# ZeayW/Multimodal-fusion-based-Pre-routing-Timing-Prediction-

Hardware: AMD Instinct MI355X
Metric: train-step samples/sec (higher is better)
Workload: dtype bf16; 1 GPU; config B: 8 designs/step/GPU, 65536-node netlist, 64 levels, 256x256 tile, 1350 endpoints/design, UNet(max), bf16 operands / fp32 accumulate on the MFMA-bound contractions; U-Net activations and their gradients stored bf16, netlist tensors, statistics, parameters and gradients fp32; nodes=65536, levels=64, tile=256, endpoints_per_design=1350, cone_pruning=False, parallelism=dp1 (designs sharded, one all-reduce of the flat gradient per step), launch=one HIP graph replay per step (Adam inside)

## Files before the change

multimodal-fusion-based-pre-routing-timing-prediction-_amd/csrc/mlp2_bf16.hip:

```cpp
#include <stdlib.h>
#include "mlp_tile_bf16.h"
#include "fold_gather.h"

namespace mmft {

constexpr int L2_BM = 32;

struct Mlp2Bf16Args {
  const float* x1;
  long long ldx1;
  const int* rows;
  int n;
  const unsigned short* w1;
  const float* b1;
  const unsigned short* w2;
  const float* b2;
  const float* mask;
  long long ldmask;
  float* hid_out;
  long long ldhid;
  int hid16;
  float* out;
  long long ldout;
  int add_act, relu_out;
  const unsigned char* active;
};

__global__ void __launch_bounds__(512) mlp2_rows_bf16_kernel(Mlp2Bf16Args a) {
  __shared__ __attribute__((aligned(16))) unsigned short xs[L2_BM * L2_XS];
  __shared__ __attribute__((aligned(16))) unsigned short hs[L2_BM * L2_HS];
  const int tid = threadIdx.x, lane = tid & 63, wave = tid >> 6;
  const int m0 = blockIdx.x * L2_BM;
  auto live_row = [&](int r) -> bool { return m0 + r < a.n && (!a.active || a.active[a.rows[m0 + r]]); };
  if (a.active) {
    int any = 0;
    if (tid < L2_BM) any = live_row(tid) ? 1 : 0;
    if (!__syncthreads_or(any)) return;
  }
  const int r16 = lane & 15, q = lane >> 4;

  bf16x8 w1f[2][4], w2f[8];
  load_w1_frags(w1f, a.w1, wave, r16, q);
  load_w2_frags(w2f, a.w2, wave, r16, q);
  {
    const int r = tid >> 4, k8 = (tid & 15) * 8;
    f32x4 v0 = {0.f, 0.f, 0.f, 0.f}, v1 = v0;
    if (live_row(r)) {
      const float* p = a.x1 + (long long)a.rows[m0 + r] * a.ldx1 + k8;
      v0 = *reinterpret_cast<const f32x4*>(p);
      v1 = *reinterpret_cast<const f32x4*>(p + 4);
    }
    u32x4 pk = {pack_bf16(v0.x, v0.y), pack_bf16(v0.z, v0.w), pack_bf16(v1.x, v1.y), pack_bf16(v1.z, v1.w)};
    *reinterpret_cast<u32x4*>(xs + r * L2_XS + k8) = pk;
  }
  __syncthreads();

  f32x4 acc1[2][2];
  tile_layer1<4, 2>(acc1, w1f, xs, L2_XS, r16, q);
#pragma unroll
  for (int i = 0; i < 2; ++i)
#pragma unroll
    for (int j = 0; j < 2; ++j) {
      const int m = i * 16 + r16, nn = wave * 32 + j * 16 + q * 4;
      f32x4 v = acc1[i][j];
      const bool live = live_row(m);
      const long long row = live ? (long long)a.rows[m0 + m] : 0;
      if (a.mask) {
        f32x4 mk = {0.f, 0.f, 0.f, 0.f};
        if (live) mk = hid_load4(a.mask, row * a.ldmask + nn, a.hid16);
        v = relu_mask4(v, mk);
      } else {
        if (a.b1) v += *reinterpret_cast<const f32x4*>(a.b1 + nn);
        v = relu4(v);
      }
      st_bf16x4(hs + m * L2_HS + nn, v);
      if (a.hid_out && live) hid_store4(a.hid_out, row * a.ldhid + nn, v, a.hid16);
    }
  __syncthreads();

  f32x4 acc2[2];
#pragma unroll
  for (int i = 0; i < 2; ++i) acc2[i] = tile_layer2(w2f, hs, L2_HS, r16, q, i);
#pragma unroll
  for (int i = 0; i < 2; ++i) {
    const int m = i * 16 + r16;
    if (!live_row(m)) continue;
    const int nn = wave * 16 + q * 4;
    float* o = a.out + (long long)a.rows[m0 + m] * a.ldout + nn;
    f32x4 v = acc2[i];
    if (a.b2) v += *reinterpret_cast<const f32x4*>(a.b2 + nn);
    if (a.add_act) v += *reinterpret_cast<const f32x4*>(o);
    if (a.relu_out) v = relu4(v);
    *reinterpret_cast<f32x4*>(o) = v;
  }
}

template <bool KEEP>
struct Kept {};
template <>
struct Kept<true> {
  float *A, *LSE;
  float* hid_out;
  long long ldhid;
  int hid16;
};

struct LevelFwdCommon {
  float* h;
  const float* pre;
  long long ld;
  const int *in_ptr, *in_idx, *ic_ptr, *ic_idx, *ic_drv;
  int net_row0, n_net;
  const int* rows;
  int cell_row0, n_cell;
  const unsigned short *w1, *w2;
  const float *b1, *b2;
  int relu;
  const unsigned char* active;
  int cell_tiles;
};

template <bool KEEP>
struct LevelFwdArgs : LevelFwdCommon, Kept<KEEP> {};

template <bool KEEP>
__global__ void __launch_bounds__(512) level_fwd_bf16_kernel(LevelFwdArgs<KEEP> a) {
  constexpr int BM = 16;
  __shared__ __attribute__((aligned(16))) unsigned short xs[BM * L2_XS];
  __shared__ __attribute__((aligned(16))) unsigned short hs[BM * L2_HS];
  const int tid = threadIdx.x, lane = tid & 63, wave = tid >> 6;
  const FoldSrc fs{a.h, a.pre, a.ld, a.in_ptr, a.in_idx, a.ic_idx, a.ic_drv, a.net_row0, a.n_net, a.relu};
  if ((int)blockIdx.x >= a.cell_tiles) {
    const long long total = (long long)a.n_net * 32;
    for (long long t = (long long)(blockIdx.x - a.cell_tiles) * 512 + tid; t < total;
         t += (long long)(gridDim.x - a.cell_tiles) * 512) {
      const int u = a.net_row0 + (int)(t >> 5), c = ((int)t & 31) * 4;
      if (a.active && !a.active[u]) continue;
      *reinterpret_cast<f32x4*>(a.h + (long long)u * a.ld + c) = fold_net_value(fs, u, c);
    }
    return;
  }
  const int m0 = blockIdx.x * BM;
  auto row_of = [&](int r) -> int { return a.rows ? a.rows[m0 + r] : a.cell_row0 + m0 + r; };
  auto live_row = [&](int r) -> bool { return m0 + r < a.n_cell && (!a.active || a.active[row_of(r)]); };
  if (a.active) {
    int any = 0;
    if (tid < BM) any = live_row(tid) ? 1 : 0;
    if (!__syncthreads_or(any)) return;
  }
  const int r16 = lane & 15, q = lane >> 4;
  bf16x8 w1f[2][4], w2f[8];
  load_w1_frags(w1f, a.w1, wave, r16, q);

  {
    const int r = tid >> 5, c = (tid & 31) * 4;
    f32x4 av = {0.f, 0.f, 0.f, 0.f};
    if (live_row(r)) {
      const int v = row_of(r);
      const int e0 = a.ic_ptr[v], e1 = a.ic_ptr[v + 1];
      SoftAccT<true> sa;
      sa.init();
      fold_gather_edges(fs, e0, e1, 1, c, sa);
      [[maybe_unused]] f32x4 lv = {0.f, 0.f, 0.f, 0.f};
      if (e1 > e0) {
#pragma unroll
        for (int j = 0; j < 4; ++j) {
          av[j] = sa.acc[j] / sa.s[j];
          if constexpr (KEEP) lv[j] = sa.mx[j] + fg_log<true>(sa.s[j]);
        }
      }
      if constexpr (KEEP) {
        *reinterpret_cast<f32x4*>(a.A + (long long)v * a.ld + c) = av;
        *reinterpret_cast<f32x4*>(a.LSE + (long long)v * a.ld + c) = lv;
      }
    }
    st_bf16x4(xs + r * L2_XS + c, av);
  }
  load_w2_frags(w2f, a.w2, wave, r16, q);
  __syncthreads();

  f32x4 acc1[1][2];
  tile_layer1<4, 1>(acc1, w1f, xs, L2_XS, r16, q);
#pragma unroll
  for (int j = 0; j < 2; ++j) {
    const int nn = wave * 32 + j * 16 + q * 4;
    f32x4 v = acc1[0][j];
    if (a.b1) v += *reinterpret_cast<const f32x4*>(a.b1 + nn);
    v = relu4(v);
    st_bf16x4(hs + r16 * L2_HS + nn, v);
    if constexpr (KEEP) {
      if (a.hid_out && live_row(r16)) hid_store4(a.hid_out, (long long)row_of(r16) * a.ldhid + nn, v, a.hid16);
    }
  }
  __syncthreads();
  if (!live_row(r16)) return;
  const int nn = wave * 16 + q * 4;
  float* o = a.h + (long long)row_of(r16) * a.ld + nn;
  f32x4 v = tile_layer2(w2f, hs, L2_HS, r16, q, 0);
  if (a.b2) v += *reinterpret_cast<const f32x4*>(a.b2 + nn);
  v += *reinterpret_cast<const f32x4*>(o);
  if (a.relu) v = relu4(v);
  *reinterpret_cast<f32x4*>(o) = v;
}

struct LevelSlotsCommon {
  float* h;
  const float* pre;
  long long ld;
  const int* slots;
  const int* net_drv;
  int net_row0, n_net, cell_row0, n_cell;
  const unsigned short *w1, *w2;
  const float *b1, *b2;
  int relu;
  const unsigned char* active;
  int cell_tiles;
};

template <bool KEEP>
struct LevelSlotsArgs : LevelSlotsCommon, Kept<KEEP> {};

template <int RB, bool KEEP>
__global__ void __launch_bounds__(512) level_fwd_slots_kernel(LevelSlotsArgs<KEEP> a) {
  constexpr int BM = 16 * RB;
  __shared__ __attribute__((aligned(16))) unsigned short xs[BM * L2_XS];
  __shared__ __attribute__((aligned(16))) unsigned short hs[BM * L2_HS];
  const int tid = threadIdx.x, lane = tid & 63, wave = tid >> 6;
  const int r16 = lane & 15, q = lane >> 4;
  const int b = blockIdx.x, gr = tid >> 5, gc = (tid & 31) * 4;
  const bool has_cell = b < a.cell_tiles;
  const int m0 = b * BM;
  int nd[RB];
  f32x4 npre[RB];
  bool net_ok[RB], live[RB];
  int hrow[RB][4], prow[RB][4];
#pragma unroll
  for (int rb = 0; rb < RB; ++rb) {
    const int nrow = b * BM + gr + 16 * rb, u = a.net_row0 + nrow;
    net_ok[rb] = nrow < a.n_net && (!a.active || a.active[u]);
    nd[rb] = -1;
    npre[rb] = f32x4{0.f, 0.f, 0.f, 0.f};
    if (net_ok[rb]) {
      nd[rb] = a.net_drv[u];
      npre[rb] = *reinterpret_cast<const f32x4*>(a.pre + (long long)u * a.ld + gc);
    }
    const int v = a.cell_row0 + m0 + gr + 16 * rb;
    live[rb] = has_cell && m0 + gr + 16 * rb < a.n_cell && (!a.active || a.active[v]);
#pragma unroll
    for (int k = 0; k < 4; ++k) hrow[rb][k] = prow[rb][k] = -1;
    if (live[rb]) {
      const int4 s0 = *reinterpret_cast<const int4*>(a.slots + (long long)v * 8);
      const int4 s1 = *reinterpret_cast<const int4*>(a.slots + (long long)v * 8 + 4);
      hrow[rb][0] = s0.x; hrow[rb][1] = s0.y; hrow[rb][2] = s0.z; hrow[rb][3] = s0.w;
      prow[rb][0] = s1.x; prow[rb][1] = s1.y; prow[rb][2] = s1.z; prow[rb][3] = s1.w;
    }
  }
  bf16x8 w1f[2][4], w2f[8];
  bool elive[RB];
  f32x4 hold[RB];
#pragma unroll
  for (int rb = 0; rb < RB; ++rb) {
    const int ev = a.cell_row0 + m0 + r16 + 16 * rb;
    elive[rb] = has_cell && m0 + r16 + 16 * rb < a.n_cell && (!a.active || a.active[ev]);
    hold[rb] = f32x4{0.f, 0.f, 0.f, 0.f};
  }
  if (has_cell) {
    load_w1_frags(w1f, a.w1, wave, r16, q);
#pragma unroll
    for (int rb = 0; rb < RB; ++rb)
      if (elive[rb]) hold[rb] = *reinterpret_cast<const f32x4*>(a.h + (long long)(a.cell_row0 + m0 + r16 + 16 * rb) * a.ld + wave * 16 + q * 4);
  }
#pragma unroll
  for (int rb = 0; rb < RB; ++rb)
    if (net_ok[rb]) {
      const int u = a.net_row0 + b * BM + gr + 16 * rb;
      f32x4 hd = {0.f, 0.f, 0.f, 0.f};
      if (nd[rb] >= 0) hd = *reinterpret_cast<const f32x4*>(a.h + (long long)nd[rb] * a.ld + gc);
      *reinterpret_cast<f32x4*>(a.h + (long long)u * a.ld + gc) = fg_finish_net(hd, npre[rb], a.relu);
    }
  if (!has_cell) return;
  if (a.active) {
    int any = 0;
    if (tid < BM) any = (m0 + tid < a.n_cell && a.active[a.cell_row0 + m0 + tid]) ? 1 : 0;
    if (!__syncthreads_or(any)) return;
  }
#pragma unroll
  for (int rb = 0; rb < RB; ++rb) {
    const int v = a.cell_row0 + m0 + gr + 16 * rb;
    f32x4 av = {0.f, 0.f, 0.f, 0.f};
    if (live[rb]) {
      const int h0 = hrow[rb][0] >= 0 ? hrow[rb][0] : v;
      f32x4 xa[4], xp[4];
#pragma unroll
      for (int k = 0; k < 4; ++k) {
        xa[k] = *reinterpret_cast<const f32x4*>(a.h + (long long)(hrow[rb][k] >= 0 ? hrow[rb][k] : h0) * a.ld + gc);
        xp[k] = *reinterpret_cast<const f32x4*>(a.pre + (long long)(prow[rb][k] >= 0 ? prow[rb][k] : a.net_row0) * a.ld + gc);
      }
      SoftAccT<true> sa;
      sa.init();
#pragma unroll
      for (int k = 0; k < 4; ++k) {
        const f32x4 x = prow[rb][k] >= 0 ? fg_finish_net(xa[k], xp[k], a.relu) : xa[k];
        SoftAccT<true> nx = sa;
        nx.add(x);
        const bool ok = hrow[rb][k] >= 0;
#pragma unroll
        for (int j = 0; j < 4; ++j) {
          sa.mx[j] = ok ? nx.mx[j] : sa.mx[j];
          sa.s[j] = ok ? nx.s[j] : sa.s[j];
          sa.acc[j] = ok ? nx.acc[j] : sa.acc[j];
        }
      }
      [[maybe_unused]] f32x4 lv = {0.f, 0.f, 0.f, 0.f};
      if (hrow[rb][0] >= 0) {
#pragma unroll
        for (int j = 0; j < 4; ++j) {
          av[j] = sa.acc[j] / sa.s[j];
          if constexpr (KEEP) lv[j] = sa.mx[j] + fg_log<true>(sa.s[j]);
        }
      }
      if constexpr (KEEP) {
        *reinterpret_cast<f32x4*>(a.A + (long long)v * a.ld + gc) = av;
        *reinterpret_cast<f32x4*>(a.LSE + (long long)v * a.ld + gc) = lv;
      }
    }
    st_bf16x4(xs + (gr + 16 * rb) * L2_XS + gc, av);
  }
  load_w2_frags(w2f, a.w2, wave, r16, q);
  __syncthreads();
  f32x4 acc1[RB][2];
  tile_layer1<4, RB>(acc1, w1f, xs, L2_XS, r16, q);
#pragma unroll
  for (int rb = 0; rb < RB; ++rb)
#pragma unroll
    for (int j = 0; j < 2; ++j) {
      const int nn = wave * 32 + j * 16 + q * 4;
      f32x4 hv = acc1[rb][j];
      if (a.b1) hv += *reinterpret_cast<const f32x4*>(a.b1 + nn);
      hv = relu4(hv);
      st_bf16x4(hs + (r16 + 16 * rb) * L2_HS + nn, hv);
      if constexpr (KEEP) {
        if (a.hid_out && elive[rb])
          hid_store4(a.hid_out, (long long)(a.cell_row0 + m0 + r16 + 16 * rb) * a.ldhid + nn, hv, a.hid16);
      }
    }
  __syncthreads();
#pragma unroll
  for (int rb = 0; rb < RB; ++rb) {
    f32x4 o = tile_layer2(w2f, hs, L2_HS, r16, q, rb);
    if (elive[rb]) {
      const int nn = wave * 16 + q * 4;
      if (a.b2) o += *reinterpret_cast<const f32x4*>(a.b2 + nn);
      o += hold[rb];
      if (a.relu) o = relu4(o);
      *reinterpret_cast<f32x4*>(a.h + (long long)(a.cell_row0 + m0 + r16 + 16 * rb) * a.ld + nn) = o;
    }
  }
}

struct LevelBwdPairArgs {
  float* G;
  const float* h;
  const float* A;
  const float* LSE;
  float* DA;
  long long ld;
  const unsigned char* own;
  const int* tiles;
  const int* on_ptr;
  int sink_shift;
  const int* cslots;
  const int* oc_ptr;
  const int* oc_idx;
  float* scratch;
  int* counters;
  int relu, has_mlp;
  const unsigned short* w1;
  const unsigned short* w2;
  const float* mask;
  long long ldmask;
  float* hid_out;
  long long ldhid;
  int hid16;
};

__global__ void __launch_bounds__(512) level_bwd_pair_kernel(LevelBwdPairArgs a) {
  constexpr int BM = 32, SC = 32, SGP = L2_K1 + 4;
  __shared__ __attribute__((aligned(16))) float sg[SC * SGP];
  __shared__ __attribute__((aligned(16))) unsigned short xs[BM * L2_XS];
  __shared__ __attribute__((aligned(16))) unsigned short hs[BM * L2_HS];
  __shared__ int s_last;
  const int tid = threadIdx.x, lane = tid & 63, wave = tid >> 6;
  const int r16 = lane & 15, q = lane >> 4;
  const int gr = tid >> 5, gc = (tid & 31) * 4;
  const int4 t0 = *reinterpret_cast<const int4*>(a.tiles + 8 * (long long)blockIdx.x);
  const int4 t1 = *reinterpret_cast<const int4*>(a.tiles + 8 * (long long)blockIdx.x + 4);
  const int v0 = t0.x, nd = t0.y, part = t0.z, parts = t0.w, sbase = t1.x, cidx = t1.y;
  const int e0 = t1.z, e1 = t1.w;
  const f32x4 zero = {0.f, 0.f, 0.f, 0.f};
  int ps[2] = {0, 0}, pe[2] = {0, 0};
  f32x4 acc[2] = {zero, zero}, hv[2] = {zero, zero};
#pragma unroll
  for (int d = 0; d < 2; ++d) {
    const int v = v0 + gr + 16 * d;
    if (gr + 16 * d < nd) {
      ps[d] = a.on_ptr[v];
      pe[d] = a.on_ptr[v + 1];
      hv[d] = *reinterpret_cast<const f32x4*>(a.h + (long long)v * a.ld + gc);
      const bool mine_v = (!a.own || a.own[v]) && !parts;
      acc[d] = *reinterpret_cast<const f32x4*>(a.G + (long long)v * a.ld + gc);
#pragma unroll
      for (int j = 0; j < 4; ++j) acc[d][j] = mine_v ? acc[d][j] : 0.f;
    }
  }
  for (int c0 = e0; c0 < e1; c0 += SC) {
    const int cend = c0 + SC < e1 ? c0 + SC : e1;
    int e = c0 + gr;
    int4 cs = {-1, -1, -1, -1};
    f32x4 hw = zero, gw = zero;
    unsigned char mine = 0;
    if (e < cend) {
      const int w = e + a.sink_shift;
      cs = *reinterpret_cast<const int4*>(a.cslots + (long long)w * 4);
      hw = *reinterpret_cast<const f32x4*>(a.h + (long long)w * a.ld + gc);
      mine = a.own ? a.own[w] : (unsigned char)1;
      gw = *reinterpret_cast<const f32x4*>(a.G + (long long)w * a.ld + gc);
    }
#pragma unroll 1
    for (; e < cend; e += 16) {
      const int w = e + a.sink_shift;
      const int c[4] = {cs.x, cs.y, cs.z, cs.w};
      const int c0row = c[0] >= 0 ? c[0] : w;
      f32x4 da[4], aa[4], ll[4];
#pragma unroll
      for (int k = 0; k < 4; ++k) {
        const long long o = (long long)(c[k] >= 0 ? c[k] : c0row) * a.ld + gc;
        da[k] = *reinterpret_cast<const f32x4*>(a.DA + o);
        aa[k] = *reinterpret_cast<const f32x4*>(a.A + o);
        ll[k] = *reinterpret_cast<const f32x4*>(a.LSE + o);
      }
      f32x4 g = gw;
      const f32x4 hcur = hw;
#pragma unroll
      for (int j = 0; j < 4; ++j) g[j] = mine ? g[j] : 0.f;
      const int en = e + 16;
      if (en < cend) {
        const int wn = en + a.sink_shift;
        cs = *reinterpret_cast<const int4*>(a.cslots + (long long)wn * 4);
        hw = *reinterpret_cast<const f32x4*>(a.h + (long long)wn * a.ld + gc);
        mine = a.own ? a.own[wn] : (unsigned char)1;
        gw = *reinterpret_cast<const f32x4*>(a.G + (long long)wn * a.ld + gc);
      }
#pragma unroll
      for (int k = 0; k < 4; ++k) {
        if (!__builtin_amdgcn_ballot_w64(c[k] >= 0)) continue;
#pragma unroll
        for (int j = 0; j < 4; ++j) g[j] = c[k] >= 0 ? cell_consumer_term<true>(g[j], da[k][j], hcur[j], ll[k][j], aa[k][j]) : g[j];
      }
      if (c[3] <= -2) {
        const int x1 = a.oc_ptr[w + 1];
        for (int x = -2 - c[3]; x < x1; ++x) {
          const long long o = (long long)a.oc_idx[x] * a.ld + gc;
          const f32x4 d2 = *reinterpret_cast<const f32x4*>(a.DA + o), a2 = *reinterpret_cast<const f32x4*>(a.A + o),
                      l2 = *reinterpret_cast<const f32x4*>(a.LSE + o);
#pragma unroll
          for (int j = 0; j < 4; ++j) g[j] = cell_consumer_term<true>(g[j], d2[j], hcur[j], l2[j], a2[j]);
        }
      }
      if (a.relu) {
#pragma unroll
        for (int j = 0; j < 4; ++j) g[j] = hcur[j] > 0.f ? g[j] : 0.f;
      }
      *reinterpret_cast<f32x4*>(a.G + (long long)w * a.ld + gc) = g;
      *reinterpret_cast<f32x4*>(sg + (e - c0) * SGP + gc) = g;
    }
    __syncthreads();
#pragma unroll
    for (int d = 0; d < 2; ++d) {
      const int lo = ps[d] > c0 ? ps[d] : c0, hi = pe[d] < cend ? pe[d] : cend;
      for (int x = lo; x < hi; ++x) acc[d] += *reinterpret_cast<const f32x4*>(sg + (x - c0) * SGP + gc);
    }
    __syncthreads();
  }
  if (parts) {
    if (gr == 0) {
      float* p = a.scratch + (long long)(sbase + part) * L2_K1 + gc;
#pragma unroll
      for (int j = 0; j < 4; ++j) __hip_atomic_store(p + j, acc[0][j], __ATOMIC_RELAXED, __HIP_MEMORY_SCOPE_AGENT);
      __builtin_amdgcn_fence(__ATOMIC_RELEASE, "agent");
    }
    __syncthreads();
    if (tid == 0) {
      const int old = __hip_atomic_fetch_add(a.counters + cidx, 1, __ATOMIC_RELAXED, __HIP_MEMORY_SCOPE_AGENT);
      s_last = old == parts - 1;
      if (old == parts - 1) __hip_atomic_store(a.counters + cidx, 0, __ATOMIC_RELAXED, __HIP_MEMORY_SCOPE_AGENT);
    }
    __syncthreads();
    if (!s_last) return;
    __builtin_amdgcn_fence(__ATOMIC_ACQUIRE, "agent");
    if (gr == 0) {
      acc[0] = zero;
      if (!a.own || a.own[v0]) acc[0] = *reinterpret_cast<const f32x4*>(a.G + (long long)v0 * a.ld + gc);
      for (int i = 0; i < parts; ++i) {
        const float* p = a.scratch + (long long)(sbase + i) * L2_K1 + gc;
#pragma unroll
        for (int j = 0; j < 4; ++j) acc[0][j] += __hip_atomic_load(p + j, __ATOMIC_RELAXED, __HIP_MEMORY_SCOPE_AGENT);
      }
    }
  }
#pragma unroll
  for (int d = 0; d < 2; ++d) {
    if (a.relu) {
#pragma unroll
      for (int j = 0; j < 4; ++j) acc[d][j] = hv[d][j] > 0.f ? acc[d][j] : 0.f;
    }
    if (gr + 16 * d < nd) *reinterpret_cast<f32x4*>(a.G + (long long)(v0 + gr + 16 * d) * a.ld + gc) = acc[d];
  }
  if (!a.has_mlp) return;
#pragma unroll
  for (int d = 0; d < 2; ++d) st_bf16x4(xs + (gr + 16 * d) * L2_XS + gc, acc[d]);
  const int nrb = nd > 16 ? 2 : 1;
  bf16x8 w1f[2][4], w2f[8];
  load_w1_frags(w1f, a.w1, wave, r16, q);
  f32x4 mk[2][2];
#pragma unroll
  for (int i = 0; i < 2; ++i)
#pragma unroll
    for (int j = 0; j < 2; ++j) {
      mk[i][j] = zero;
      if (r16 + 16 * i < nd)
        mk[i][j] = hid_load4(a.mask, (long long)(v0 + r16 + 16 * i) * a.ldmask + wave * 32 + j * 16 + q * 4, a.hid16);
    }
  load_w2_frags(w2f, a.w2, wave, r16, q);
  __syncthreads();
  f32x4 acc1[2][2];
  tile_layer1<4, 2>(acc1, w1f, xs, L2_XS, r16, q, nrb);
#pragma unroll
  for (int i = 0; i < 2; ++i) {
    if (i >= nrb) continue;
    const int row = r16 + 16 * i;
#pragma unroll
    for (int j = 0; j < 2; ++j) {
      const int nn = wave * 32 + j * 16 + q * 4;
      const f32x4 hvv = relu_mask4(acc1[i][j], mk[i][j]);
      st_bf16x4(hs + row * L2_HS + nn, hvv);
      if (a.hid_out && row < nd) hid_store4(a.hid_out, (long long)(v0 + row) * a.ldhid + nn, hvv, a.hid16);
    }
  }
  __syncthreads();
#pragma unroll
  for (int i = 0; i < 2; ++i) {
    if (i >= nrb) continue;
    const f32x4 acc2 = tile_layer2(w2f, hs, L2_HS, r16, q, i);
    if (r16 + 16 * i < nd) *reinterpret_cast<f32x4*>(a.DA + (long long)(v0 + r16 + 16 * i) * a.ld + wave * 16 + q * 4) = acc2;
  }
}

__global__ void __launch_bounds__(256) pack_bf16_kernel(const float* __restrict__ src, long long ld, int R, int C,
                                                        unsigned short* __restrict__ dst, int transpose) {
  const long long total = (long long)R * C;
  for (long long i = (long long)blockIdx.x * blockDim.x + threadIdx.x; i < total; i += (long long)gridDim.x * blockDim.x) {
    int dr = (int)(i / (transpose ? R : C)), dc = (int)(i - (long long)dr * (transpose ? R : C));
    float v = transpose ? src[(long long)dc * ld + dr] : src[(long long)dr * ld + dc];
    dst[i] = (unsigned short)(pack_bf16(v, 0.f) & 0xffff);
  }
}

}

using namespace mmft;

static bool opt_aligned16(const void* p, long long ld = 0) { return !p || (aligned16(p) && ld % 4 == 0); }

extern "C" int mmft_pack_bf16(const float* src, long long ld, int R, int C, void* dst, int transpose, int device,
                              void* stream) {
  MMFT_REQUIRE(src && dst && R > 0 && C > 0 && ld >= C, "pack_bf16: bad args");
  DeviceGuard dg(device);
  hipLaunchKernelGGL(pack_bf16_kernel, dim3(ew_grid((long long)R * C)), dim3(256), 0, (hipStream_t)stream, src, ld, R, C,
                     (unsigned short*)dst, transpose);
  return check_launch("pack_bf16");
}

extern "C" int mmft_mlp2_rows_bf16(const float* x1, long long ldx1, const int* rows, int n, const void* w1_bf16,
                                   const float* b1, const void* w2_bf16, const float* b2, const float* mask,
                                   long long ldmask, float* hid_out, long long ldhid, float* out, long long ldout,
                                   int add_act, int relu_out, int K1, int HD, int D2, const unsigned char* active, int hid_bf16,
                                   int device, void* stream) {
  MMFT_REQUIRE(x1 && rows && w1_bf16 && w2_bf16 && out, "mlp2_rows_bf16: null pointer");
  if (K1 != L2_K1 || HD != L2_HD || D2 != L2_D2) {
    set_error("mlp2_rows_bf16: only %d -> %d -> %d is fused (got %d -> %d -> %d)", L2_K1, L2_HD, L2_D2, K1, HD, D2);
    return MMFT_ERR_UNSUPPORTED;
  }
  MMFT_REQUIRE(n >= 0, "mlp2_rows_bf16: negative row count");
  MMFT_REQUIRE(ldx1 % 4 == 0 && ldout % 4 == 0 && aligned16(x1) && aligned16(out) && aligned16(w1_bf16) && aligned16(w2_bf16) &&
                   opt_aligned16(b1) && opt_aligned16(b2),
               "mlp2_rows_bf16: operands must be 16-byte aligned");
  MMFT_REQUIRE(opt_aligned16(mask, ldmask), "mlp2_rows_bf16: mask alignment");
  MMFT_REQUIRE(opt_aligned16(hid_out, ldhid), "mlp2_rows_bf16: hid_out alignment");
  if (n == 0) return MMFT_OK;
  DeviceGuard dg(device);
  Mlp2Bf16Args a{x1, ldx1, rows, n, (const unsigned short*)w1_bf16, b1, (const unsigned short*)w2_bf16, b2, mask, ldmask,
                 hid_out, ldhid, hid_bf16 ? 1 : 0, out, ldout, add_act, relu_out, active};
  const double fl = 2.0 * n * ((double)K1 * HD + (double)HD * D2), by = 4.0 * n * ((double)K1 + 2.0 * HD + 2.0 * D2);
  MMFT_LAUNCH(mask ? "mlp2_rows_bf16_kernel<bwd>" : "mlp2_rows_bf16_kernel<fwd>", fl, by, mlp2_rows_bf16_kernel,
              dim3(cdiv(n, L2_BM)), dim3(512), (hipStream_t)stream, a);
  return check_launch("mlp2_rows_bf16");
}

static bool kept_given(const Kept<true>& k) { return k.A && k.LSE; }
static bool kept_given(const Kept<false>&) { return true; }
static bool kept_aligned(const Kept<true>& k) { return opt_aligned16(k.A) && opt_aligned16(k.LSE) && opt_aligned16(k.hid_out, k.ldhid); }
static bool kept_aligned(const Kept<false>&) { return true; }
static double level_mlp_flops(int n_cell) { return 2.0 * n_cell * ((double)L2_K1 * L2_HD + (double)L2_HD * L2_D2); }

template <bool KEEP>
static int launch_level_fwd_bf16(LevelFwdArgs<KEEP> a, int D, long long alg_bytes, int device, void* stream) {
  constexpr const char* fn = KEEP ? "level_fwd_bf16" : "level_fwd_bf16_infer";
  MMFT_REQUIRE(D == L2_K1, "%s: D must be %d", fn, L2_K1);
  MMFT_REQUIRE(a.n_net >= 0 && a.n_cell >= 0 && a.net_row0 >= 0 && a.cell_row0 >= 0, "%s: negative row count / offset", fn);
  if (a.n_net + a.n_cell == 0) return MMFT_OK;
  MMFT_REQUIRE(a.h && a.pre && a.in_ptr && a.ic_ptr && (a.n_cell == 0 || (kept_given(a) && a.w1 && a.w2)), "%s: null pointer", fn);
  MMFT_REQUIRE(a.ld >= D && a.ld % 4 == 0 && aligned16(a.h) && aligned16(a.pre) && kept_aligned(a) && opt_aligned16(a.w1) &&
                   opt_aligned16(a.w2) && opt_aligned16(a.b1) && opt_aligned16(a.b2),
               "%s: operands must be 16-byte aligned", fn);
  DeviceGuard dg(device);
  constexpr int LV_BM = 16;
  a.cell_tiles = cdiv(a.n_cell, LV_BM);
  int net_blocks = cdiv((long long)a.n_net * 32, 512);
  if (net_blocks > 1024) net_blocks = 1024;
  MMFT_LAUNCH(KEEP ? "level_fwd_bf16_kernel" : "level_fwd_bf16_infer_kernel", level_mlp_flops(a.n_cell),
              alg_bytes > 0 ? (double)alg_bytes : 0.0, level_fwd_bf16_kernel<KEEP>, dim3(a.cell_tiles + net_blocks), dim3(512),
              (hipStream_t)stream, a);
  return check_launch(fn);
}

extern "C" int mmft_level_fwd_bf16(float* h, const float* pre, long long ld, int D, const int* in_net_indptr,
                                   const int* in_net_indices, const int* in_cell_indptr, const int* in_cell_indices,
                                   int net_row0, int n_net, const int* cell_rows, int cell_row0, int n_cell, float* A,
                                   float* LSE, const void* w1_bf16, const float* b1, const void* w2_bf16, const float* b2,
                                   float* hid_out, long long ldhid, int relu, const unsigned char* active,
                                   const int* in_cell_driver, long long alg_bytes, int hid_bf16, int device, void* stream) {
  return launch_level_fwd_bf16<true>({{h, pre, ld, in_net_indptr, in_net_indices, in_cell_indptr, in_cell_indices, in_cell_driver,
                                       net_row0, n_net, cell_rows, cell_row0, n_cell, (const unsigned short*)w1_bf16,
                                       (const unsigned short*)w2_bf16, b1, b2, relu, active, 0},
                                      {A, LSE, hid_out, ldhid, hid_bf16 ? 1 : 0}},
                                     D, alg_bytes, device, stream);
}

extern "C" int mmft_level_fwd_bf16_infer(float* h, const float* pre, long long ld, int D, const int* in_net_indptr,
                                         const int* in_net_indices, const int* in_cell_indptr, const int* in_cell_indices,
                                         int net_row0, int n_net, const int* cell_rows, int cell_row0, int n_cell,
                                         const void* w1_bf16, const float* b1, const void* w2_bf16, const float* b2, int relu,
                                         const unsigned char* active, const int* in_cell_driver, long long alg_bytes, int device,
                                         void* stream) {
  return launch_level_fwd_bf16<false>({{h, pre, ld, in_net_indptr, in_net_indices, in_cell_indptr, in_cell_indices, in_cell_driver,
                                        net_row0, n_net, cell_rows, cell_row0, n_cell, (const unsigned short*)w1_bf16,
                                        (const unsigned short*)w2_bf16, b1, b2, relu, active, 0},
                                       {}},
                                      D, alg_bytes, device, stream);
}

static int level_slots_rb(int n_net, int n_cell) {
  static const int rb_env = getenv("MMFT_FWD_RB") ? atoi(getenv("MMFT_FWD_RB")) : 0;
  const int rows_max = n_cell > n_net ? n_cell : n_net;
  return rb_env ? rb_env : (rows_max >= 32 * 192 ? 2 : 1);
}

template <bool KEEP>
static int launch_level_fwd_slots(LevelSlotsArgs<KEEP> a, int D, long long alg_bytes, int device, void* stream) {
  constexpr const char* fn = KEEP ? "level_fwd_slots" : "level_fwd_slots_infer";
  MMFT_REQUIRE(D == L2_K1, "%s: D must be %d", fn, L2_K1);
  MMFT_REQUIRE(a.n_net >= 0 && a.n_cell >= 0 && a.net_row0 >= 0 && a.cell_row0 >= 0, "%s: negative row count / offset", fn);
  if (a.n_net + a.n_cell == 0) return MMFT_OK;
  MMFT_REQUIRE(a.h && a.pre && a.slots && a.net_drv && (a.n_cell == 0 || (kept_given(a) && a.w1 && a.w2)), "%s: null pointer", fn);
  MMFT_REQUIRE(a.ld >= D && a.ld % 4 == 0 && aligned16(a.h) && aligned16(a.pre) && aligned16(a.slots) && kept_aligned(a) &&
                   opt_aligned16(a.w1) && opt_aligned16(a.w2) && opt_aligned16(a.b1) && opt_aligned16(a.b2),
               "%s: operands must be 16-byte aligned", fn);
  DeviceGuard dg(device);
  const bool rb2 = level_slots_rb(a.n_net, a.n_cell) == 2;
  const int bm = rb2 ? 32 : 16, net_tiles = cdiv(a.n_net, bm);
  a.cell_tiles = cdiv(a.n_cell, bm);
  MMFT_LAUNCH(KEEP ? "level_fwd_slots_kernel" : "level_fwd_slots_infer_kernel", level_mlp_flops(a.n_cell),
              alg_bytes > 0 ? (double)alg_bytes : 0.0, (rb2 ? level_fwd_slots_kernel<2, KEEP> : level_fwd_slots_kernel<1, KEEP>),
              dim3(a.cell_tiles > net_tiles ? a.cell_tiles : net_tiles), dim3(512), (hipStream_t)stream, a);
  return check_launch(fn);
}

extern "C" int mmft_level_fwd_slots(float* h, const float* pre, long long ld, int D, const int* slots, const int* net_driver,
                                    int net_row0, int n_net, int cell_row0, int n_cell, float* A, float* LSE, const void* w1_bf16,
                                    const float* b1, const void* w2_bf16, const float* b2, float* hid_out, long long ldhid, int relu,
                                    const unsigned char* active, long long alg_bytes, int hid_bf16, int device, void* stream) {
  return launch_level_fwd_slots<true>({{h, pre, ld, slots, net_driver, net_row0, n_net, cell_row0, n_cell, (const unsigned short*)w1_bf16,
                                        (const unsigned short*)w2_bf16, b1, b2, relu, active, 0},
                                       {A, LSE, hid_out, ldhid, hid_bf16 ? 1 : 0}},
                                      D, alg_bytes, device, stream);
}

extern "C" int mmft_level_fwd_slots_infer(float* h, const float* pre, long long ld, int D, const int* slots, const int* net_driver,
                                          int net_row0, int n_net, int cell_row0, int n_cell, const void* w1_bf16, const float* b1,
                                          const void* w2_bf16, const float* b2, int relu, const unsigned char* active,
                                          long long alg_bytes, int device, void* stream) {
  return launch_level_fwd_slots<false>({{h, pre, ld, slots, net_driver, net_row0, n_net, cell_row0, n_cell, (const unsigned short*)w1_bf16,
                                         (const unsigned short*)w2_bf16, b1, b2, relu, active, 0},
                                        {}},
                                       D, alg_bytes, device, stream);
}

extern "C" int mmft_level_bwd_pair(float* G, const float* h, const float* A, const float* LSE, float* DA, long long ld, int D, int N,
                                   const unsigned char* own_mask, const int* tiles, int ntiles, const int* out_net_indptr,
                                   int sink_shift, const int* cslots, const int* out_cell_indptr,
                                   const int* out_cell_indices, float* scratch, int* counters, int relu, int has_mlp,
                                   const void* w1_bf16, const void* w2_bf16, const float* mask, long long ldmask, float* hid_out,
                                   long long ldhid, long long alg_bytes, int hid_bf16, int device, void* stream) {
  MMFT_REQUIRE(D == L2_K1, "level_bwd_pair: D must be %d", L2_K1);
  MMFT_REQUIRE(ntiles >= 0 && N > 0, "level_bwd_pair: negative tile count");
  if (ntiles == 0) return MMFT_OK;
  MMFT_REQUIRE(G && h && A && LSE && DA && tiles && out_net_indptr && cslots && out_cell_indptr && out_cell_indices && scratch && counters,
               "level_bwd_pair: null pointer");
  MMFT_REQUIRE(!has_mlp || (w1_bf16 && w2_bf16 && mask), "level_bwd_pair: the MLP part needs both weight packs and the saved hidden rows");
  MMFT_REQUIRE(ld >= D && ld % 4 == 0 && aligned16(G) && aligned16(h) && aligned16(A) && aligned16(LSE) && aligned16(DA) &&
                   aligned16(cslots) && aligned16(tiles) && aligned16(scratch) && opt_aligned16(w1_bf16) &&
                   opt_aligned16(w2_bf16) && opt_aligned16(mask, ldmask) && opt_aligned16(hid_out, ldhid),
               "level_bwd_pair: operands must be 16-byte aligned");
  DeviceGuard dg(device);
  LevelBwdPairArgs a{G, h, A, LSE, DA, ld, own_mask, tiles, out_net_indptr, sink_shift, cslots, out_cell_indptr, out_cell_indices,
                     scratch, counters, relu, has_mlp, (const unsigned short*)w1_bf16, (const unsigned short*)w2_bf16, mask, ldmask,
                     hid_out, ldhid, hid_bf16 ? 1 : 0};
  MMFT_LAUNCH("level_bwd_pair_kernel", 0.0, alg_bytes > 0 ? (double)alg_bytes : 0.0, level_bwd_pair_kernel, dim3(ntiles), dim3(512),
              (hipStream_t)stream, a);
  return check_launch("level_bwd_pair");
}
```

multimodal-fusion-based-pre-routing-timing-prediction-_amd/csrc/mlp_tile_bf16.h:

```cpp
#pragma once
#include "gemm_bf16.h"

namespace mmft {

constexpr int L2_K1 = 128, L2_HD = 256, L2_D2 = 128;
constexpr int L2_XS = L2_K1 + 8, L2_HS = L2_HD + 8;

__device__ __forceinline__ f32x4 relu4(f32x4 v) {
  v.x = v.x > 0.f ? v.x : 0.f; v.y = v.y > 0.f ? v.y : 0.f;
  v.z = v.z > 0.f ? v.z : 0.f; v.w = v.w > 0.f ? v.w : 0.f;
  return v;
}
__device__ __forceinline__ f32x4 relu_mask4(f32x4 v, f32x4 mk) {
  v.x = mk.x > 0.f ? v.x : 0.f; v.y = mk.y > 0.f ? v.y : 0.f;
  v.z = mk.z > 0.f ? v.z : 0.f; v.w = mk.w > 0.f ? v.w : 0.f;
  return v;
}
__device__ __forceinline__ void st_bf16x4(unsigned short* p, f32x4 v) {
  const unsigned lo = pack_bf16(v.x, v.y), hi = pack_bf16(v.z, v.w);
  *reinterpret_cast<unsigned long long*>(p) = ((unsigned long long)hi << 32) | lo;
}

__device__ __forceinline__ void hid_store4(float* base, long long off, f32x4 v, int hid16) {
  if (hid16) {
    const unsigned lo = pack_bf16(v.x, v.y), hi = pack_bf16(v.z, v.w);
    *reinterpret_cast<unsigned long long*>(reinterpret_cast<unsigned short*>(base) + off) = ((unsigned long long)hi << 32) | lo;
  } else {
    *reinterpret_cast<f32x4*>(base + off) = v;
  }
}
__device__ __forceinline__ f32x4 hid_load4(const float* base, long long off, int hid16) {
  if (!hid16) return *reinterpret_cast<const f32x4*>(base + off);
  const unsigned long long u = *reinterpret_cast<const unsigned long long*>(reinterpret_cast<const unsigned short*>(base) + off);
  const unsigned lo = (unsigned)u, hi = (unsigned)(u >> 32);
  return f32x4{__uint_as_float(lo << 16), __uint_as_float(lo & 0xffff0000u), __uint_as_float(hi << 16), __uint_as_float(hi & 0xffff0000u)};
}

__device__ __forceinline__ void load_w1_frags(bf16x8 (&f)[2][4], const unsigned short* w1, int wave, int r16, int q) {
#pragma unroll
  for (int j = 0; j < 2; ++j)
#pragma unroll
    for (int ks = 0; ks < 4; ++ks)
      f[j][ks] = *reinterpret_cast<const bf16x8*>(w1 + (long long)(wave * 32 + j * 16 + r16) * L2_K1 + ks * 32 + q * 8);
}
__device__ __forceinline__ void load_w2_frags(bf16x8 (&f)[8], const unsigned short* w2, int wave, int r16, int q) {
#pragma unroll
  for (int ks = 0; ks < 8; ++ks)
    f[ks] = *reinterpret_cast<const bf16x8*>(w2 + (long long)(wave * 16 + r16) * L2_HD + ks * 32 + q * 8);
}

template <int KS, int RB>
__device__ __forceinline__ void tile_layer1(f32x4 (&acc)[RB][2], const bf16x8 (&w1f)[2][KS], const unsigned short* xs, int stride,
                                            int r16, int q, int nrb = RB) {
#pragma unroll
  for (int i = 0; i < RB; ++i)
#pragma unroll
    for (int j = 0; j < 2; ++j) acc[i][j] = f32x4{0.f, 0.f, 0.f, 0.f};
#pragma unroll
  for (int ks = 0; ks < KS; ++ks)
#pragma unroll
    for (int i = 0; i < RB; ++i) {
      if (i >= nrb) continue;
      const bf16x8 xf = *reinterpret_cast<const bf16x8*>(xs + (i * 16 + r16) * stride + ks * 32 + q * 8);
#pragma unroll
      for (int j = 0; j < 2; ++j) acc[i][j] = __builtin_amdgcn_mfma_f32_16x16x32_bf16(w1f[j][ks], xf, acc[i][j], 0, 0, 0);
    }
}

__device__ __forceinline__ f32x4 tile_layer2(const bf16x8 (&w2f)[8], const unsigned short* hs, int stride, int r16, int q, int i) {
  f32x4 acc = {0.f, 0.f, 0.f, 0.f};
#pragma unroll
  for (int ks = 0; ks < 8; ++ks) {
    const bf16x8 hf = *reinterpret_cast<const bf16x8*>(hs + (i * 16 + r16) * stride + ks * 32 + q * 8);
    acc = __builtin_amdgcn_mfma_f32_16x16x32_bf16(w2f[ks], hf, acc, 0, 0, 0);
  }
  return acc;
}

}
```

Before: 2626 designs/s.

## Hoist gathers and bias loads ahead of compute in level forward slots kernel

Restructures the level-forward slots kernel to issue its independent global loads up front. It clamps row indices so loads are unconditional, batches the active-mask reads, and prefetches slot tables, net driver rows and all gathered h/pre rows for every row block before the softmax fold. Bias vectors are loaded once into registers in all three MLP kernels, and the A/LSE stores are deferred until after the layer-1 staging. The aim is more memory-level parallelism and fewer dependent round-trips to memory, at the cost of higher register pressure from the xa/xp arrays, which may reduce occupancy.

```diff
diff --git a/multimodal-fusion-based-pre-routing-timing-prediction-_amd/csrc/mlp2_bf16.hip b/multimodal-fusion-based-pre-routing-timing-prediction-_amd/csrc/mlp2_bf16.hip
--- a/multimodal-fusion-based-pre-routing-timing-prediction-_amd/csrc/mlp2_bf16.hip
+++ b/multimodal-fusion-based-pre-routing-timing-prediction-_amd/csrc/mlp2_bf16.hip
@@ -40,8 +40,10 @@
   const int r16 = lane & 15, q = lane >> 4;
 
   bf16x8 w1f[2][4], w2f[8];
+  f32x4 b1v[2], b2v;
   load_w1_frags(w1f, a.w1, wave, r16, q);
   load_w2_frags(w2f, a.w2, wave, r16, q);
+  load_bias_frags(b1v, b2v, a.mask ? nullptr : a.b1, a.b2, wave, q);
   {
     const int r = tid >> 4, k8 = (tid & 15) * 8;
     f32x4 v0 = {0.f, 0.f, 0.f, 0.f}, v1 = v0;
@@ -70,7 +72,7 @@
         if (live) mk = hid_load4(a.mask, row * a.ldmask + nn, a.hid16);
         v = relu_mask4(v, mk);
       } else {
-        if (a.b1) v += *reinterpret_cast<const f32x4*>(a.b1 + nn);
+        if (a.b1) v += b1v[j];
         v = relu4(v);
       }
       st_bf16x4(hs + m * L2_HS + nn, v);
@@ -88,7 +90,7 @@
     const int nn = wave * 16 + q * 4;
     float* o = a.out + (long long)a.rows[m0 + m] * a.ldout + nn;
     f32x4 v = acc2[i];
-    if (a.b2) v += *reinterpret_cast<const f32x4*>(a.b2 + nn);
+    if (a.b2) v += b2v;
     if (a.add_act) v += *reinterpret_cast<const f32x4*>(o);
     if (a.relu_out) v = relu4(v);
     *reinterpret_cast<f32x4*>(o) = v;
@@ -150,7 +152,9 @@
   }
   const int r16 = lane & 15, q = lane >> 4;
   bf16x8 w1f[2][4], w2f[8];
+  f32x4 b1v[2], b2v;
   load_w1_frags(w1f, a.w1, wave, r16, q);
+  load_bias_frags(b1v, b2v, a.b1, a.b2, wave, q);
 
   {
     const int r = tid >> 5, c = (tid & 31) * 4;
@@ -185,7 +189,7 @@
   for (int j = 0; j < 2; ++j) {
     const int nn = wave * 32 + j * 16 + q * 4;
     f32x4 v = acc1[0][j];
-    if (a.b1) v += *reinterpret_cast<const f32x4*>(a.b1 + nn);
+    if (a.b1) v += b1v[j];
     v = relu4(v);
     st_bf16x4(hs + r16 * L2_HS + nn, v);
     if constexpr (KEEP) {
@@ -197,7 +201,7 @@
   const int nn = wave * 16 + q * 4;
   float* o = a.h + (long long)row_of(r16) * a.ld + nn;
   f32x4 v = tile_layer2(w2f, hs, L2_HS, r16, q, 0);
-  if (a.b2) v += *reinterpret_cast<const f32x4*>(a.b2 + nn);
+  if (a.b2) v += b2v;
   v += *reinterpret_cast<const f32x4*>(o);
   if (a.relu) v = relu4(v);
   *reinterpret_cast<f32x4*>(o) = v;
@@ -230,77 +234,113 @@
   const int b = blockIdx.x, gr = tid >> 5, gc = (tid & 31) * 4;
   const bool has_cell = b < a.cell_tiles;
   const int m0 = b * BM;
+  const int rowx = has_cell ? a.cell_row0 + m0 : a.net_row0 + m0;
+  bool net_ok[RB], live[RB], elive[RB];
+  int urow[RB], vrow[RB], evrow[RB];
+#pragma unroll
+  for (int rb = 0; rb < RB; ++rb) {
+    net_ok[rb] = m0 + gr + 16 * rb < a.n_net;
+    live[rb] = has_cell && m0 + gr + 16 * rb < a.n_cell;
+    elive[rb] = has_cell && m0 + r16 + 16 * rb < a.n_cell;
+    urow[rb] = net_ok[rb] ? a.net_row0 + m0 + gr + 16 * rb : rowx;
+    vrow[rb] = live[rb] ? a.cell_row0 + m0 + gr + 16 * rb : rowx;
+    evrow[rb] = elive[rb] ? a.cell_row0 + m0 + r16 + 16 * rb : rowx;
+  }
+  if (a.active) {
+    unsigned char an[RB], ag[RB], ae[RB];
+#pragma unroll
+    for (int rb = 0; rb < RB; ++rb) {
+      an[rb] = a.active[urow[rb]];
+      ag[rb] = a.active[vrow[rb]];
+      ae[rb] = a.active[evrow[rb]];
+    }
+#pragma unroll
+    for (int rb = 0; rb < RB; ++rb) {
+      net_ok[rb] = net_ok[rb] & (an[rb] != 0);
+      live[rb] = live[rb] & (ag[rb] != 0);
+      elive[rb] = elive[rb] & (ae[rb] != 0);
+    }
+  }
+  const f32x4 zero = {0.f, 0.f, 0.f, 0.f};
   int nd[RB];
-  f32x4 npre[RB];
-  bool net_ok[RB], live[RB];
+  f32x4 npre[RB], nhd[RB];
+  auto request_net_tables = [&]() {
+#pragma unroll
+    for (int rb = 0; rb < RB; ++rb) nd[rb] = a.net_drv[urow[rb]];
+#pragma unroll
+    for (int rb = 0; rb < RB; ++rb) npre[rb] = *reinterpret_cast<const f32x4*>(a.pre + (long long)urow[rb] * a.ld + gc);
+  };
+  auto request_net_rows = [&]() {
+#pragma unroll
+    for (int rb = 0; rb < RB; ++rb)
+      nhd[rb] = *reinterpret_cast<const f32x4*>(a.h + (long long)(net_ok[rb] && nd[rb] >= 0 ? nd[rb] : urow[rb]) * a.ld + gc);
+  };
+  auto store_net_rows = [&]() {
+#pragma unroll
+    for (int rb = 0; rb < RB; ++rb) {
+      f32x4 hd;
+#pragma unroll
+      for (int j = 0; j < 4; ++j) hd[j] = nd[rb] >= 0 ? nhd[rb][j] : 0.f;
+      if (net_ok[rb]) *reinterpret_cast<f32x4*>(a.h + (long long)urow[rb] * a.ld + gc) = fg_finish_net(hd, npre[rb], a.relu);
+    }
+  };
+  if (!has_cell) {
+    request_net_tables();
+    request_net_rows();
+    store_net_rows();
+    return;
+  }
+  int4 s0[RB], s1[RB];
+#pragma unroll
+  for (int rb = 0; rb < RB; ++rb) {
+    s0[rb] = *reinterpret_cast<const int4*>(a.slots + (long long)vrow[rb] * 8);
+    s1[rb] = *reinterpret_cast<const int4*>(a.slots + (long long)vrow[rb] * 8 + 4);
+  }
+  request_net_tables();
+  f32x4 hold[RB], b1v[2], b2v;
+#pragma unroll
+  for (int rb = 0; rb < RB; ++rb)
+    hold[rb] = *reinterpret_cast<const f32x4*>(a.h + (long long)evrow[rb] * a.ld + wave * 16 + q * 4);
+  load_bias_frags(b1v, b2v, a.b1, a.b2, wave, q);
+  request_net_rows();
+  if (a.active) {
+    store_net_rows();
+    int any = 0;
+#pragma unroll
+    for (int rb = 0; rb < RB; ++rb) any |= live[rb] ? 1 : 0;
+    if (!__syncthreads_or(any)) return;
+  }
   int hrow[RB][4], prow[RB][4];
+  f32x4 xa[RB][4], xp[RB][4];
 #pragma unroll
   for (int rb = 0; rb < RB; ++rb) {
-    const int nrow = b * BM + gr + 16 * rb, u = a.net_row0 + nrow;
-    net_ok[rb] = nrow < a.n_net && (!a.active || a.active[u]);
-    nd[rb] = -1;
-    npre[rb] = f32x4{0.f, 0.f, 0.f, 0.f};
-    if (net_ok[rb]) {
-      nd[rb] = a.net_drv[u];
-      npre[rb] = *reinterpret_cast<const f32x4*>(a.pre + (long long)u * a.ld + gc);
-    }
-    const int v = a.cell_row0 + m0 + gr + 16 * rb;
-    live[rb] = has_cell && m0 + gr + 16 * rb < a.n_cell && (!a.active || a.active[v]);
-#pragma unroll
-    for (int k = 0; k < 4; ++k) hrow[rb][k] = prow[rb][k] = -1;
+    const int hs4[4] = {s0[rb].x, s0[rb].y, s0[rb].z, s0[rb].w}, ps4[4] = {s1[rb].x, s1[rb].y, s1[rb].z, s1[rb].w};
+#pragma unroll
+    for (int k = 0; k < 4; ++k) {
+      hrow[rb][k] = live[rb] ? hs4[k] : -1;
+      prow[rb][k] = live[rb] ? ps4[k] : -1;
+    }
+    const int h0 = hrow[rb][0] >= 0 ? hrow[rb][0] : vrow[rb];
+#pragma unroll
+    for (int k = 0; k < 4; ++k) {
+      xa[rb][k] = *reinterpret_cast<const f32x4*>(a.h + (long long)(hrow[rb][k] >= 0 ? hrow[rb][k] : h0) * a.ld + gc);
+      xp[rb][k] = *reinterpret_cast<const f32x4*>(a.pre + (long long)(prow[rb][k] >= 0 ? prow[rb][k] : a.net_row0) * a.ld + gc);
+    }
+  }
+  bf16x8 w1f[2][4], w2f[8];
+  if (RB == 1) load_w1_frags(w1f, a.w1, wave, r16, q);
+  if (!a.active) store_net_rows();
+  [[maybe_unused]] f32x4 kav[RB], klv[RB];
+#pragma unroll
+  for (int rb = 0; rb < RB; ++rb) {
+    if (RB > 1 && rb == 1) load_w1_frags(w1f, a.w1, wave, r16, q);
+    f32x4 av = zero;
     if (live[rb]) {
-      const int4 s0 = *reinterpret_cast<const int4*>(a.slots + (long long)v * 8);
-      const int4 s1 = *reinterpret_cast<const int4*>(a.slots + (long long)v * 8 + 4);
-      hrow[rb][0] = s0.x; hrow[rb][1] = s0.y; hrow[rb][2] = s0.z; hrow[rb][3] = s0.w;
-      prow[rb][0] = s1.x; prow[rb][1] = s1.y; prow[rb][2] = s1.z; prow[rb][3] = s1.w;
-    }
-  }
-  bf16x8 w1f[2][4], w2f[8];
-  bool elive[RB];
-  f32x4 hold[RB];
-#pragma unroll
-  for (int rb = 0; rb < RB; ++rb) {
-    const int ev = a.cell_row0 + m0 + r16 + 16 * rb;
-    elive[rb] = has_cell && m0 + r16 + 16 * rb < a.n_cell && (!a.active || a.active[ev]);
-    hold[rb] = f32x4{0.f, 0.f, 0.f, 0.f};
-  }
-  if (has_cell) {
-    load_w1_frags(w1f, a.w1, wave, r16, q);
-#pragma unroll
-    for (int rb = 0; rb < RB; ++rb)
-      if (elive[rb]) hold[rb] = *reinterpret_cast<const f32x4*>(a.h + (long long)(a.cell_row0 + m0 + r16 + 16 * rb) * a.ld + wave * 16 + q * 4);
-  }
-#pragma unroll
-  for (int rb = 0; rb < RB; ++rb)
-    if (net_ok[rb]) {
-      const int u = a.net_row0 + b * BM + gr + 16 * rb;
-      f32x4 hd = {0.f, 0.f, 0.f, 0.f};
-      if (nd[rb] >= 0) hd = *reinterpret_cast<const f32x4*>(a.h + (long long)nd[rb] * a.ld + gc);
-      *reinterpret_cast<f32x4*>(a.h + (long long)u * a.ld + gc) = fg_finish_net(hd, npre[rb], a.relu);
-    }
-  if (!has_cell) return;
-  if (a.active) {
-    int any = 0;
-    if (tid < BM) any = (m0 + tid < a.n_cell && a.active[a.cell_row0 + m0 + tid]) ? 1 : 0;
-    if (!__syncthreads_or(any)) return;
-  }
-#pragma unroll
-  for (int rb = 0; rb < RB; ++rb) {
-    const int v = a.cell_row0 + m0 + gr + 16 * rb;
-    f32x4 av = {0.f, 0.f, 0.f, 0.f};
-    if (live[rb]) {
-      const int h0 = hrow[rb][0] >= 0 ? hrow[rb][0] : v;
-      f32x4 xa[4], xp[4];
-#pragma unroll
-      for (int k = 0; k < 4; ++k) {
-        xa[k] = *reinterpret_cast<const f32x4*>(a.h + (long long)(hrow[rb][k] >= 0 ? hrow[rb][k] : h0) * a.ld + gc);
-        xp[k] = *reinterpret_cast<const f32x4*>(a.pre + (long long)(prow[rb][k] >= 0 ? prow[rb][k] : a.net_row0) * a.ld + gc);
-      }
       SoftAccT<true> sa;
       sa.init();
 #pragma unroll
       for (int k = 0; k < 4; ++k) {
-        const f32x4 x = prow[rb][k] >= 0 ? fg_finish_net(xa[k], xp[k], a.relu) : xa[k];
+        const f32x4 x = prow[rb][k] >= 0 ? fg_finish_net(xa[rb][k], xp[rb][k], a.relu) : xa[rb][k];
         SoftAccT<true> nx = sa;
         nx.add(x);
         const bool ok = hrow[rb][k] >= 0;
@@ -311,7 +351,7 @@
           sa.acc[j] = ok ? nx.acc[j] : sa.acc[j];
         }
       }
-      [[maybe_unused]] f32x4 lv = {0.f, 0.f, 0.f, 0.f};
+      [[maybe_unused]] f32x4 lv = zero;
       if (hrow[rb][0] >= 0) {
 #pragma unroll
         for (int j = 0; j < 4; ++j) {
@@ -319,14 +359,20 @@
           if constexpr (KEEP) lv[j] = sa.mx[j] + fg_log<true>(sa.s[j]);
         }
       }
-      if constexpr (KEEP) {
-        *reinterpret_cast<f32x4*>(a.A + (long long)v * a.ld + gc) = av;
-        *reinterpret_cast<f32x4*>(a.LSE + (long long)v * a.ld + gc) = lv;
-      }
-    }
+      if constexpr (KEEP) klv[rb] = lv;
+    }
+    if constexpr (KEEP) kav[rb] = av;
     st_bf16x4(xs + (gr + 16 * rb) * L2_XS + gc, av);
   }
   load_w2_frags(w2f, a.w2, wave, r16, q);
+  if constexpr (KEEP) {
+#pragma unroll
+    for (int rb = 0; rb < RB; ++rb)
+      if (live[rb]) {
+        *reinterpret_cast<f32x4*>(a.A + (long long)vrow[rb] * a.ld + gc) = kav[rb];
+        *reinterpret_cast<f32x4*>(a.LSE + (long long)vrow[rb] * a.ld + gc) = klv[rb];
+      }
+  }
   __syncthreads();
   f32x4 acc1[RB][2];
   tile_layer1<4, RB>(acc1, w1f, xs, L2_XS, r16, q);
@@ -336,12 +382,11 @@
     for (int j = 0; j < 2; ++j) {
       const int nn = wave * 32 + j * 16 + q * 4;
       f32x4 hv = acc1[rb][j];
-      if (a.b1) hv += *reinterpret_cast<const f32x4*>(a.b1 + nn);
+      if (a.b1) hv += b1v[j];
       hv = relu4(hv);
       st_bf16x4(hs + (r16 + 16 * rb) * L2_HS + nn, hv);
       if constexpr (KEEP) {
-        if (a.hid_out && elive[rb])
-          hid_store4(a.hid_out, (long long)(a.cell_row0 + m0 + r16 + 16 * rb) * a.ldhid + nn, hv, a.hid16);
+        if (a.hid_out && elive[rb]) hid_store4(a.hid_out, (long long)evrow[rb] * a.ldhid + nn, hv, a.hid16);
       }
     }
   __syncthreads();
@@ -350,10 +395,10 @@
     f32x4 o = tile_layer2(w2f, hs, L2_HS, r16, q, rb);
     if (elive[rb]) {
       const int nn = wave * 16 + q * 4;
-      if (a.b2) o += *reinterpret_cast<const f32x4*>(a.b2 + nn);
+      if (a.b2) o += b2v;
       o += hold[rb];
       if (a.relu) o = relu4(o);
-      *reinterpret_cast<f32x4*>(a.h + (long long)(a.cell_row0 + m0 + r16 + 16 * rb) * a.ld + nn) = o;
+      *reinterpret_cast<f32x4*>(a.h + (long long)evrow[rb] * a.ld + nn) = o;
     }
   }
 }
diff --git a/multimodal-fusion-based-pre-routing-timing-prediction-_amd/csrc/mlp_tile_bf16.h b/multimodal-fusion-based-pre-routing-timing-prediction-_amd/csrc/mlp_tile_bf16.h
--- a/multimodal-fusion-based-pre-routing-timing-prediction-_amd/csrc/mlp_tile_bf16.h
+++ b/multimodal-fusion-based-pre-routing-timing-prediction-_amd/csrc/mlp_tile_bf16.h
@@ -49,6 +49,15 @@
     f[ks] = *reinterpret_cast<const bf16x8*>(w2 + (long long)(wave * 16 + r16) * L2_HD + ks * 32 + q * 8);
 }
 
+__device__ __forceinline__ void load_bias_frags(f32x4 (&b1v)[2], f32x4& b2v, const float* b1, const float* b2, int wave, int q) {
+  b1v[0] = b1v[1] = b2v = f32x4{0.f, 0.f, 0.f, 0.f};
+  if (b1) {
+#pragma unroll
+    for (int j = 0; j < 2; ++j) b1v[j] = *reinterpret_cast<const f32x4*>(b1 + wave * 32 + j * 16 + q * 4);
+  }
+  if (b2) b2v = *reinterpret_cast<const f32x4*>(b2 + wave * 16 + q * 4);
+}
+
 template <int KS, int RB>
 __device__ __forceinline__ void tile_layer1(f32x4 (&acc)[RB][2], const bf16x8 (&w1f)[2][KS], const unsigned short* xs, int stride,
                                             int r16, int q, int nrb = RB) {
```

New measurement: 2644 designs/s, median of 6. Within noise of the previous version (+0.7%).
